# gt1/daccord

Measured on AMD Instinct MI355X. Metric: corrected Mbase/s (whole node), synthetic 20x PacBio piles, higher is better.
Workload: dtype u64+f64

## Files before the change

### daccord_amd/csrc/capi.hip

```cpp
#include <hip/hip_runtime.h>
#include <vector>
#include <string>
#include <cstring>
#include <cstdio>
#include <cstdlib>
#include <new>
#include "../../include/daccord_hip.h"
#include "batch_plan.hpp"
#include "host_tables.hpp"
#include "window_kernels.hpp"
#include "trace_kernel.hpp"
#include "vote_kernel.hpp"
#include "emit_record.hpp"

using namespace dacc;


struct PrepBatch
{
	DevOvl const * ovl; uint64_t novl; uint8_t const * trace; uint32_t trace_bytes;
	uint32_t * blk_ovl; uint32_t * blk_b0;
};

__global__ void k_prep(PrepBatch B)
// ... 528 lines not shown
		WB.pregen = 0;
		for ( uint32_t i = 0; i < TIER_NSTAGES; ++i ) c->st[i].ran = false;
		if ( TP.usefast && TP.anytier() )
		{
			HIPCHK(hipMemsetAsync(c->d_pregen.p,0,((BP.nwindows+31)/32+1)*sizeof(uint32_t),s));
			HIPCHK(hipMemsetAsync(c->d_pregen2.p,0,((BP.nwindows+31)/32+1)*sizeof(uint32_t),s));
			HIPCHK(hipMemsetAsync(c->d_pregenlist.p,0,sizeof(uint32_t),s));
			for ( int i = 0; i < TIER_NSLOTS; ++i ) HIPCHK(hipMemsetAsync(c->d_retry[i].p,0,sizeof(uint32_t),s));
			if ( BP.ovl.size() )
			{
				hipLaunchKernelGGL(k_prescan,dim3((BP.ovl.size()+3)/4),dim3(256),0,s,c->d_ovl.p,static_cast<uint64_t>(BP.ovl.size()),c->d_ovl_pile.p,c->d_piles.p,c->d_wt_b.p,c->d_wt_e.p,c->d_pregen.p,c->d_pregen2.p,TP.widetier ? 128u : 64u);
				hipLaunchKernelGGL(k_prescan_lists,dim3(((BP.nwindows+31)/32+255)/256),dim3(256),0,s,c->d_pregen.p,c->d_pregen2.p,static_cast<uint64_t>(BP.nwindows),c->d_pregenlist.p,
					TP.slot1_long ? c->d_retry[0].p : static_cast<uint32_t *>(0),c->d_wout.p);
			}
			HIPCHK(hipEventRecord(c->evPrescan,s));
			FastBatch FL; FL.W = WB; FL.W.arena = c->d_arena2.p; FL.W.prof = 0; FL.W.pregen = 0; FL.F = BP.ftierL; FL.dpsq_vst = c->d_vst.p; FL.retry = 0; FL.gearly = 0; FL.gslab = 0; FL.gstride = 0; FL.tab32 = c->d_tab32.p; FL.hand = 0; FL.handctr = 0; FL.handcap = 0; FL.handwords = 0;
#if defined(DACC_LEDGER)
			FL.ledger = 0;
#endif
			if ( !TP.ok[ID_LONG] ) FL.F.ldsbytes = 0;
			auto const launchLong = [&](uint32_t const * const lst, uint32_t & nlist, hipEvent_t const filled) -> int
			{
				nlist = 0;
				HIPCHK(hipStreamWaitEvent(c->stream2,filled,0));
				HIPCHK(hipMemcpyAsync(&nlist,lst,sizeof(uint32_t),hipMemcpyDeviceToHost,c->stream2));
				HIPCHK(hipStreamSynchronize(c->stream2));
				if ( !nlist ) return DACC_OK;
				uint32_t const grid = nlist < c->early_grid ? nlist : c->early_grid;
				(void)hipGetLastError();
				hipLaunchKernelGGL(k_window_long,dim3(grid),dim3(64),FL.F.ldsbytes,c->stream2,FL,c->d_err.p,lst);
				if ( FL.F.ldsbytes && hipGetLastError() != hipSuccess )
// ... 8 lines not shown
			HIPCHK(hipMemsetAsync(c->d_gearly.p,0,sizeof(uint32_t),s));
			HIPCHK(hipMemsetAsync(c->d_handctr.p,0,sizeof(uint32_t),s));
			bool early = false;
			HIPCHK(hipMemsetAsync(c->d_work.p,0,WORK_WORDS*sizeof(uint32_t),s));
			auto const work = [&](uint32_t const off) { return (c->sched&1) ? c->d_work.p+off : static_cast<uint32_t *>(0); };
			uint32_t const * list = 0; int lastslot = -1;
			FastBatch FZ;
			for ( uint32_t slot = 0; slot < TIER_NSLOTS; ++slot )
			{
				if ( TP.slotok(slot) )
				{
					int const m = TIER_MAIN[slot];
					FastBatch FB; FB.W = WB; FB.F = BP.stageCaps(m); FB.dpsq_vst = c->d_vst.p; FB.retry = c->d_retry[slot].p;
					if ( (slot > 0 && TP.late_long) || TP.widetier ) FB.W.pregen = c->d_pregen2.p;
					FB.gslab = c->d_gslab.p; FB.gstride = FB.F.gbytes; FB.tab32 = c->d_tab32.p;
					FB.hand = c->handcap ? c->d_hand.p : static_cast<uint64_t *>(0); FB.handctr = c->d_handctr.p; FB.handcap = c->handcap; FB.handwords = TP.handwords;
#if defined(DACC_LEDGER)
					{ char const * lm = getenv("DACC_LEDGER_MASK"); FB.ledger = lm ? static_cast<uint32_t>(strtoul(lm,0,0)) : 0u; }
#endif
					FB.gearly = early ? static_cast<uint32_t *>(0) : c->d_gearly.p;
					int fr[TIER_NSTAGES]; uint32_t nfr = 0;
					for ( int i = 0; i < m; ++i ) if ( TIER_CHAIN[i].slot == slot && TP.ok[i] && !((TIER_CHAIN[i].flags & STAGE_ADAPTIVE) && c->tier7_adapt_off) ) fr[nfr++] = i;
					bool const classed = nfr && (TIER_CHAIN[fr[0]].flags & STAGE_PREPASS);
					if ( classed ) HIPCHK(hipMemsetAsync(c->d_small.p,0,sizeof(uint32_t),s));
					for ( uint32_t k = 0; k < nfr; ++k ) HIPCHK(hipMemsetAsync(c->st[fr[k]].handon.p,0,sizeof(uint32_t),s));
					uint32_t const * in = list;
					if ( classed )
					{
						uint32_t * const mid = c->st[fr[0]].handon.p, * const big = c->st[fr[nfr-1]].handon.p;
						hipLaunchKernelGGL(k_classify,dim3((BP.nwindows+255)/256),dim3(256),0,s,WB,c->d_small.p,mid,big,c->sw.t0inst,nfr > 1 ? c->sw.t7inst : 0u);
						if ( nfr > 1 ) { HIPCHK(hipMemcpyAsync(c->d_work.p+WORK_PRE_MID,mid,sizeof(uint32_t),hipMemcpyDeviceToDevice,s)); HIPCHK(hipMemcpyAsync(c->d_work.p+WORK_PRE_BIG,big,sizeof(uint32_t),hipMemcpyDeviceToDevice,s)); }
// ... 509 lines not shown
```

### daccord_amd/csrc/fast_window.hpp

```cpp
#ifndef DACC_FAST_WINDOW_HPP
#define DACC_FAST_WINDOW_HPP
#include "wave.hpp"
#include "dev_types.hpp"
#include "arena.hpp"
#include "window_main.hpp"
#include "tier_pipeline.hpp"
#include "emit_record.hpp"

namespace dacc {

enum { WS_RETRY = 4 };
enum { FNOPAR = 0xFF };
enum { FSEQCAP = 48 };

struct FSI { uint64_t w; uint16_t left, right, current, path; };
struct FCC { uint64_t w; uint32_t o, l; };

template<int TIER> struct FastTier;
#if !defined(DACC_RCH01)
#define DACC_RCH01 2
#endif
template<> struct FastTier<1> { typedef uint8_t id_t; typedef uint8_t sid_t; enum : uint32_t { smax = 250, gw = 1, wcapg = 1024, rch = DACC_RCH01, fch = 4, fnw = 2, fnc = 40, idmax = 250, rpstcap = 256, lstr = 64, maxs = 32, precap = 1024, ncap = 776, scap = 112, lcap = 960, wcap = 1024, rccap = 144, fcap = 192, siqcap = 56, blcap = 96, seqcap = 32, psiq = 8, consrow = 64, lscrids = 2048, wide = 0, mins = 0, gmem = 0 }; };
template<> struct FastTier<0> { typedef uint8_t id_t; typedef uint8_t sid_t; enum : uint32_t { smax = 250, gw = 1, wcapg = 768, rch = DACC_RCH01, fch = 4, fnw = 2, fnc = 32, idmax = 250, rpstcap = 256, lstr = 64, maxs = 28, precap = 576, ncap = 524, scap = 88, lcap = 640, wcap = 768, rccap = 96, fcap = 128, siqcap = 56, blcap = 96, seqcap = 32, psiq = 8, consrow = 64, lscrids = 2048, wide = 0, mins = 0, gmem = 0 }; };
template<> struct FastTier<7> { typedef uint8_t id_t; typedef uint8_t sid_t; enum : uint32_t { smax = 250, gw = 1, wcapg = 896, rch = DACC_RCH01, fch = 4, fnw = 2, fnc = 32, idmax = 250, rpstcap = 256, lstr = 64, maxs = 28, precap = 704, ncap = 640, scap = 104, lcap = 800, wcap = 896, rccap = 112, fcap = 148, siqcap = 56, blcap = 96, seqcap = 32, psiq = 8, consrow = 64, lscrids = 2048, wide = 0, mins = 0, gmem = 0 }; };
// ... 383 lines not shown
	static_assert(CT::gmem == 0 || CT::gw != 0,"a layout in device memory is the gw layout");
	return C;
}

struct FastBatch
{
	WindowBatch W;
	FastCaps F;
	uint64_t const * dpsq_vst;
	uint32_t * retry;
	uint32_t * gearly;
	uint8_t * gslab;
	uint64_t gstride;
	uint32_t const * tab32;
	uint64_t * hand; uint32_t * handctr; uint32_t handcap, handwords;
#if defined(DACC_LEDGER)
	uint32_t ledger;
#endif
};

template<typename CT>
DEV void fast_load_tables(FastLds<CT> const & L, uint32_t const nrows, uint32_t const nsup, DevTables const & T, uint64_t const * vst)
{
	int const lane = wv_lane();
	for ( uint32_t i = lane; i < nsup; i += WSZ ) { L.suplo8()[i] = T.suplo[i]; L.suphi8()[i] = T.suphi[i]; }
	wv_sync();
}

#if defined(DACC_LEDGER)
#define LEDGER_REP(bit) for ( uint32_t lrep_ = 0, lrn_ = 1u + ((ledger >> (bit)) & 1u); lrep_ < lrn_; ++lrep_ )
#define LEDGER_REPX(E,bit) for ( uint32_t lrep_ = 0, lrn_ = 1u + (((E).ledger >> (bit)) & 1u); lrep_ < lrn_; ++lrep_ )
#else
#define LEDGER_REP(bit)
#define LEDGER_REPX(E,bit)
#endif
#define FW_THRES_FEAS 4294968ull
#define FW_THRES_01   429496730ull
#define FW_THRES_05   2147483648ull

#if defined(DACC_EMUL)
struct FastStats { uint32_t v[32]; void clear() { for ( int i = 0; i < 32; ++i ) v[i] = 0; } void mx(int i, uint32_t x) { if ( x > v[i] ) v[i] = x; } void add(int i, uint32_t x) { v[i] += x; } };
static FastStats g_fstats;
static inline void fstats_dump(int const tier)
{
	static FILE * sf = 0; static bool tried = false;
	if ( !tried ) { tried = true; char const * fn = getenv("DACC_EMUL_STATS"); if ( fn ) sf = fopen(fn,"w"); }
	if ( sf ) { fprintf(sf,"%d",tier); for ( int i = 0; i < 32; ++i ) fprintf(sf," %u",g_fstats.v[i]); fprintf(sf,"\n"); fflush(sf); }
}
static inline FILE * ftrav_file() { static FILE * f = 0; static bool tried = false; if ( !tried ) { tried = true; char const * fn = getenv("DACC_EMUL_TRAV"); if ( fn ) f = fopen(fn,"w"); } return f; }
#define FSTAT_MX(i,x) g_fstats.mx(i,x)
#define FSTAT_ADD(i,x) g_fstats.add(i,x)
#include <vector>
#include <algorithm>
struct FeasIters { std::vector<uint32_t> it, ln; void clear() { it.clear(); ln.clear(); } };
static FeasIters g_feasit;
static inline void feasit_dump()
{
	static FILE * f = 0; static bool tried = false;
	if ( !tried ) { tried = true; char const * fn = getenv("DACC_EMUL_FEAS"); if ( fn ) f = fopen(fn,"w"); }
	if ( !f ) { g_feasit.clear(); return; }
	std::vector<uint32_t> const & it = g_feasit.it; std::vector<uint32_t> const & ln = g_feasit.ln;
	uint64_t tot = 0, lock = 0, locksorted = 0;
// ... 33 lines not shown
	enum : bool { GW = (CT::gw != 0) };
	uint8_t * gslab;
	uint32_t const * gtab;
	struct G4 { uint32_t x, y, z, w; };
	int lane; uint32_t flags;
#if defined(DACC_LEDGER)
	uint32_t ledger;
#endif
	uint64_t * prof;
	uint32_t mao, k; uint64_t kmask;
	uint32_t npre, nlast, nn, nmfirst, nmlast;
	uint32_t n0, npool, nlinks, nwF, nwR;
	uint32_t nF, nL;

#if defined(DACC_EMUL)
	DEV void over_(uint32_t b, int line) { flags |= b; static char const * ov = getenv("DACC_EMUL_OVER"); if ( ov ) fprintf(stderr,"[over] tier maxs=%d line %d bits 0x%x nn=%u n0=%u npool=%u nF=%u nL=%u nwF=%u nwR=%u rstop=%u\n",int(CT::maxs)*10000+int(CT::ncap),line,b,nn,n0,npool,nF,nL,nwF,nwR,rstop); }
	#define over(b) over_(b,__LINE__)
#else
	DEV void over(uint32_t b) { flags |= b; }
#endif
#if defined(DACC_PROFILE) && !defined(DACC_EMUL)
	DEV void pcount(int id, uint64_t v) { if ( prof ) atomicAdd(reinterpret_cast<unsigned long long *>(prof+id),static_cast<unsigned long long>(v)); }
	DEV uint64_t pclock() { return clock64(); }
#else
	DEV void pcount(int, uint64_t) {}
	DEV uint64_t pclock() { return 0; }
#endif

#if defined(DACC_PROFILE) && !defined(DACC_EMUL)
	#define SITE_T0 uint64_t _ps = clock64();
	#define SITE_RESET { _ps = clock64(); }
// ... 32 lines not shown
		for ( uint32_t q = L.succ0()[z]; q < nn; ++q )
		{
			uint32_t const x = L.nv()[q];
			if ( x == target ) return q;
			if ( x > target ) break;
		}
		return -1;
	}
	DEV uint32_t nsucc(uint32_t z) const { return (L.sinfo()[z]>>8)&7; }
	DEV uint32_t nsuccact(uint32_t z) const { return (L.sinfo()[z]>>11)&7; }

	DEV void buildInstances()
	{
		PROFX_T0
		enum { NCH = (CT::maxs+WSZ-1)/WSZ };
#if defined(DACC_GEN_MARKS_NONE)
		enum : bool { GENMARKS = false };
#else
		enum : bool { GENMARKS = true };
#endif
		enum : bool { WIDES = FastLds<CT>::wides };
		enum : uint32_t { CLB = WIDES ? 10u : 8u, CLMASK = (1u << CLB) - 1u };
		static_assert(4u*CT::maxs <= FastLds<CT>::icap && CT::maxs <= (1u << CLB) && FastLds<CT>::icap <= (1u << (WIDES ? 16 : 24)),"compact string list: string | first slot << CLB, in the bytes of irpos");
		static_assert(!WIDES || GENMARKS,"the two-pass generation of more than 256 strings needs the marks");
		LDSQ uint8_t * const marks = L.ipos();
		LDSQ uint32_t * const clist = reinterpret_cast<LDSQ uint32_t *>(L.irpos());
		enum { NCHR = WIDES ? 1 : NCH };
		uint32_t nkc[NCHR], offc[NCHR], rkc[NCHR]; uint32_t base = 0, nl = 0;
		if constexpr ( WIDES )
		{
// ... 138 lines not shown
				p0 += dacc_popc64(m0); p1 += dacc_popc64(m1); p2 += dacc_popc64(m2); p3 += dacc_popc64(m3);
			}
			wv_sync();
			wv_sort_keys<CT::precap>(L.pre(),cnt0);
			wv_sort_keys<CT::precap>(L.pre()+o1,cnt1);
			wv_sort_keys<CT::precap>(L.pre()+o2,cnt2);
			wv_sort_keys<CT::precap>(L.pre()+o3,cnt3);
		}
		else
		wv_sort_keys<CT::precap,(CT::precap == 2048 && CT::ncap == 256)>(L.pre(),npre);
		SITE(33)
	}

	DEV void buildNodes(uint32_t const f)
	{
		uint32_t base = 0;
		for ( uint32_t c = 0; c < npre; c += WSZ )
		{
			uint32_t const i = c + lane;
			uint32_t keep = 0, e = i;
			if ( i < npre && (i == 0 || (L.pre()[i]>>32) != (L.pre()[i-1]>>32)) )
			{
				uint64_t const km = L.pre()[i]>>32;
				e = i+1;
				while ( e < npre && (L.pre()[e]>>32) == km ) ++e;
				keep = (e-i) >= f;
			}
			uint32_t tot; uint32_t const pre = wv_scan_excl(keep,tot);
			if ( keep )
			{
				uint32_t const z = base+pre;
				if ( z < CT::ncap ) { L.nv()[z] = static_cast<uint32_t>(L.pre()[i]>>32); L.nps()[z] = i; L.nfreq()[z] = (e-i) > FastLds<CT>::fqmax ? FastLds<CT>::fqmax : (e-i); if ( (e-i) > FastLds<CT>::fqmax ) over(2); }
			}
			base += tot;
		}
		nn = base;
		if ( nn > CT::ncap ) { over(2); nn = 0; }
		for ( uint32_t i = lane; i < npre; i += WSZ )
		{
			uint32_t const pos = (L.pre()[i]>>16)&0xFFFF, seq = L.pre()[i]&0xFFFF;
			uint32_t const rpos = L.slen()[seq]-pos-k;
			L.ipos()[i] = pos < nsup ? pos : nsup; L.irpos()[i] = rpos < nsup ? rpos : nsup;
		}
		wv_sync();
		if ( lane == 0 ) L.nps()[nn] = npre;
		for ( uint32_t z = lane; z < nn; z += WSZ )
		{
			uint32_t const s0 = L.nps()[z], f2 = L.nfreq()[z];
			uint32_t const lo = L.ipos()[s0], hi = L.ipos()[s0+f2-1];
			uint32_t rlo = 255, rhi = 0;
			for ( uint32_t q = 0; q < f2; ++q ) { uint32_t const r = L.irpos()[s0+q]; rlo = r < rlo ? r : rlo; rhi = r > rhi ? r : rhi; }
			uint32_t const pf = lo < nsup ? L.suplo8()[lo] : nrows, pt = hi < nsup ? L.suphi8()[hi] : nrows;
// ... 3 lines not shown
		uint32_t const kp2 = next_pow2(CT::maxs < 2 ? 2 : CT::maxs);
		base = 0;
		for ( uint32_t c = 0; c < nn; c += WSZ )
		{
			uint32_t const z = c + lane;
			uint32_t c0 = 0;
			if ( z < nn ) { uint32_t const s = L.nps()[z]; for ( uint32_t q = 0; q < L.nfreq()[z] && L.ipos()[s+q] == 0; ++q ) ++c0; }
			uint32_t tot; uint32_t const pre = wv_scan_excl(c0 ? 1 : 0,tot);
			if ( c0 && base+pre < kp2 ) L.mfirst()[base+pre] = ~((static_cast<uint64_t>(c0)<<32) | L.nv()[z]);
			base += tot;
		}
		nmfirst = base;
		if ( nmfirst > kp2 ) { over(8); nmfirst = 0; }
		uint32_t const p2 = next_pow2(nmfirst < 2 ? 2 : nmfirst);
		for ( uint32_t i = nmfirst + lane; i < p2; i += WSZ ) L.mfirst()[i] = ~0ull;
		base = 0;
		for ( uint32_t c = 0; c < nlast; c += WSZ )
		{
			uint32_t const i = c + lane;
			uint32_t const head = (i < nlast) && (i == 0 || (L.lastk()[i]>>32) != (L.lastk()[i-1]>>32));
			uint32_t tot; uint32_t const pre = wv_scan_excl(head,tot);
			if ( head )
			{
				uint32_t e = i+1;
				while ( e < nlast && (L.lastk()[e]>>32) == (L.lastk()[i]>>32) ) ++e;
				L.mlast()[base+pre] = ~((static_cast<uint64_t>(e-i)<<32) | (L.lastk()[i]>>32));
			}
			base += tot;
		}
		nmlast = base;
		uint32_t const q2 = next_pow2(nmlast < 2 ? 2 : nmlast);
		for ( uint32_t i = nmlast + lane; i < q2; i += WSZ ) L.mlast()[i] = ~0ull;
		wv_sync();
		wv_sort_keys<FastLds<CT>::keycap>(L.mfirst(),nmfirst);
		wv_sort_keys<FastLds<CT>::keycap>(L.mlast(),nmlast);
	}

	DEV void buildSuccessors(uint32_t const no)
	{
		uint32_t const lim = T.klim[(k-P.klow)*T.kln + (no < static_cast<uint32_t>(T.kln) ? no : T.kln-1)];
		for ( uint32_t z = lane; z < nn; z += WSZ )
		{
			uint32_t const masked = static_cast<uint32_t>((static_cast<uint64_t>(L.nv()[z])<<2) & kmask);
			uint32_t const s0 = lowerNode(masked);
			uint32_t k0 = 0, k1 = 0, k2 = 0, k3 = 0, n = 0;
			for ( uint32_t q = s0; q < nn && L.nv()[q] <= (masked|3); ++q )
			{
				uint32_t const kv = (static_cast<uint32_t>(L.nfreq()[q])<<8) | (L.nv()[q]&3);
				if ( n == 0 ) k0 = kv; else if ( n == 1 ) k1 = kv; else if ( n == 2 ) k2 = kv; else k3 = kv;
				++n;
// ... 15 lines not shown
			L.sinfo()[z] = order | (n<<8) | (act<<11);
		}
		wv_sync();
		sfresh = true;
	}
	DEV bool passIsDead() const
	{
		if ( nmfirst == 0 || nmlast == 0 ) return true;
		uint32_t const lastthres = ((static_cast<uint32_t>((~L.mlast()[0])>>32))*3)/4;
		uint32_t any = 0;
		for ( uint32_t i = lane; i < nmlast; i += WSZ )
		{
			uint64_t const e = ~L.mlast()[i];
			if ( static_cast<uint32_t>(e>>32) >= lastthres && findNode(static_cast<uint32_t>(e)) >= 0 ) any = 1;
		}
		return !wv_any(any);
	}
	DEV bool addNextFromHeap()
	{
		uint32_t best = 0;
		for ( uint32_t z = lane; z < nn; z += WSZ )
			if ( nsuccact(z) < nsucc(z) )
			{
				uint32_t const fq = L.nfreq()[succNode(z,nsuccact(z))];
				best = fq > best ? fq : best;
			}
		best = wv_max(best);
		if ( ! best ) return false;
		for ( uint32_t z = lane; z < nn; z += WSZ )
		{
// ... 76 lines not shown
		base = 0;
		for ( uint32_t c = 0; c < nane; c += WSZ )
		{
			uint32_t const i = c + lane;
			uint32_t ok = 0; uint32_t seqid = 0, pos = 0; uint64_t cv = 0;
			if ( i < nane )
			{
				pos = ANE[i]&0xFF; cv = ANE[i]>>8;
				for ( uint32_t j = 0; j < mao; ++j ) if ( pos + k <= L.slen()[j] ) { seqid = j; ok = 1; break; }
			}
			uint32_t tot; uint32_t const pre = wv_scan_excl(ok,tot);
			if ( ok && npre+base+pre < CT::precap ) L.pre()[npre+base+pre] = (cv<<32) | (static_cast<uint64_t>(pos)<<16) | seqid;
			base += tot;
		}
		if ( npre + base > CT::precap ) { over(1); return; }
		npre += base;
		wv_sync();
		wv_sort_keys<CT::precap>(L.pre(),npre);
	}

	DEV LDSQ uint16_t * stepTable() const { return L.xstep(); }
	DEV void computePredCounts()
	{
		LDSQ uint32_t * const cnt32 = L.xcnt32();
		LDSQ uint16_t * const stepT = stepTable();
		for ( uint32_t z = lane; 4u*z < nn; z += WSZ ) cnt32[z] = 0;
		wv_sync();
		for ( uint32_t u = lane; u < nn; u += WSZ )
		{
			uint32_t const na = nsuccact(u);
			uint32_t first = 0xFFFF;
// ... 87 lines not shown
		if ( nlinks > CT::lcap ) { over(64); n0 = 0; return; }
		wv_sync();
		for ( uint32_t q = lane; q < ns; q += WSZ )
		{
			uint32_t const len = L.tslen()[q]; uint64_t const sk = L.skey()[q];
			LDSQ uint16_t * const dst = L.links() + L.tlink()[q];
			if ( q < nslot && len <= WSLOT )
			{
				if constexpr ( GW ) { uint16_t const * src = reinterpret_cast<uint16_t const *>(gslab) + q*WSLOT; for ( uint32_t t = 0; t < len; ++t ) dst[t] = src[t]; }
				else { LDSQ uint16_t const * src = L.xwtmp() + q*WSLOT; for ( uint32_t t = 0; t < len; ++t ) dst[t] = src[t]; }
			}
			else { uint32_t ln; walkStretch(L.tfirst()[q],static_cast<uint32_t>(sk>>32),dst,ln); }
			L.tlast()[q] = static_cast<uint32_t>(sk);
		}
		wv_sync();
		uint32_t const p2 = next_pow2(ns < 2 ? 2 : ns);
		for ( uint32_t q = lane; q < p2; q += WSZ )
			L.skey()[q] = q < ns ? ((sortKey(L.tfirst()[q],L.links()[L.tlink()[q]+1],L.tslen()[q] < KFMAX ? L.tslen()[q] : KFMAX,L.tlast()[q])<<QB) | q) : ~0ull;
		wv_sync();
		wv_sort_keys<fcpow2(CT::scap)>(L.skey(),ns);
		uint32_t dup = 0;
		for ( uint32_t q = lane; q < ns; q += WSZ )
		{
			if ( q && (L.skey()[q]>>(QB+2*KF)) == (L.skey()[q-1]>>(QB+2*KF)) ) dup = 1;
			uint32_t const raw = L.skey()[q]&QMASK;
			L.sfirst()[q] = L.tfirst()[raw]; L.slast()[q] = L.tlast()[raw]; L.sslen()[q] = L.tslen()[raw]; L.slink()[q] = L.tlink()[raw];
		}
		if ( wv_any(dup) ) { over(32); n0 = 0; return; }
		n0 = ns;
		wv_sync();
		for ( uint32_t z = lane; z < nn; z += WSZ ) { L.npred()[z] = SNONE; L.lhead()[z] = SNONE; }
		for ( uint32_t q = lane; q < p2; q += WSZ ) L.skey()[q] = q < ns ? ((static_cast<uint64_t>(L.slast()[q])<<SB) | q) : ~0ull;
		wv_sync();
		for ( uint32_t q = lane; q < ns; q += WSZ ) if ( q == 0 || L.sfirst()[q-1] != L.sfirst()[q] ) L.npred()[L.sfirst()[q]] = q;
		wv_sort_keys<fcpow2(CT::scap)>(L.skey(),ns);
		for ( uint32_t q = lane; q < ns; q += WSZ )
		{
			uint64_t const e = L.skey()[q];
			L.lord()[q] = static_cast<uint32_t>(e);
			if ( q == 0 || (L.skey()[q-1]>>SB) != (e>>SB) ) L.lhead()[e>>SB] = q;
		}
		wv_sync();
	}

	DEV void makePiece(uint32_t const id, uint32_t const par, uint32_t const a, uint32_t const b)
	{
		LDSQ uint16_t const * Lk = L.links() + L.slink()[par];
		L.sfirst()[id] = Lk[a]; L.slast()[id] = Lk[b]; L.sslen()[id] = b-a+1; L.slink()[id] = L.slink()[par]+a;
	}
	DEV void findCandidatesAndPieces()
	{
		uint32_t const firstthres = nmfirst ? ((static_cast<uint32_t>((~L.mfirst()[0])>>32))*3)/4 : 0;
		uint32_t const lastthres = nmlast ? ((static_cast<uint32_t>((~L.mlast()[0])>>32))*3)/4 : 0;
		uint32_t cf = 0, cl = 0;
		while ( cf < nmfirst && static_cast<uint32_t>((~L.mfirst()[cf])>>32) >= firstthres ) ++cf;
		while ( cl < nmlast && static_cast<uint32_t>((~L.mlast()[cl])>>32) >= lastthres ) ++cl;
		nF = cf; npool = n0;
// ... 31 lines not shown
			{
				uint32_t const len = L.sslen()[s]; LDSQ uint16_t const * Lk = L.links() + L.slink()[s];
				for ( uint32_t i = 1; i+1 < len; ++i ) if ( sid[Lk[i]] != s ) multi = 1;
			}
			for ( uint32_t c = lane; c < nF; c += WSZ ) { uint32_t const z = L.fnode()[c]; if ( z != 0xFFFF && sid[z] != 0xFFFF ) { L.parF()[c] = sid[z]; L.posF()[c] = spos[z]; } }
			for ( uint32_t c = lane; c < nL; c += WSZ ) { uint32_t const z = L.lnode()[c]; if ( z != 0xFFFF && sid[z] != 0xFFFF ) { L.parL()[c] = sid[z]; L.posL()[c] = spos[z]; } }
		}
		if ( wv_any(multi) ) { over(32); return; }
		wv_sync();
		{
			uint32_t cnt = 0;
			for ( uint32_t c = 0; c < nF; ++c ) cnt += (L.parF()[c] != SNONE);
			for ( uint32_t c = 0; c < nL; ++c ) cnt += (L.parL()[c] != SNONE);
			if ( n0 + 2*cnt + 1 > CT::scap || n0 + 2*cnt + 1 > SMAX ) { over(32); return; }
		}
		{
			uint32_t id = n0;
			for ( uint32_t c0 = 0; c0 < nF + nL; c0 += WSZ )
			{
				uint32_t const c = c0 + lane;
				bool const isF = c < nF, act = c < nF + nL;
				uint32_t const ci = isF ? c : c - nF;
				uint32_t const par = act ? (isF ? L.parF()[ci] : L.parL()[ci]) : static_cast<uint32_t>(SNONE);
				bool const has = act && par != SNONE;
				uint32_t tot; uint32_t const pre = wv_scan_flag(has,tot);
				if ( has )
				{
					uint32_t const pid = id + 2*pre, pos = isF ? L.posF()[ci] : L.posL()[ci];
					if ( isF ) L.pieF()[ci] = pid; else L.pieL()[ci] = pid;
					makePiece(pid,par,0,pos); makePiece(pid+1,par,pos,L.sslen()[par]-1);
// ... 29 lines not shown
							while ( m < nm && !(L.midpar()[m] == pf && L.midA()[m] == lo && L.midB()[m] == hi) ) ++m;
							if ( m < nm ) continue;
							if ( nm < MIDCAP ) { L.midpar()[nm] = pf; L.midA()[nm] = lo; L.midB()[nm] = hi; }
							++nm;
						}
					}
				}
				wv_sync();
				nm = wv_bcast(nm,0);
				if ( nm > MIDCAP || npool + nm > CT::scap || npool + nm > SMAX ) { over(32); return; }
				for ( uint32_t m = lane; m < nm; m += WSZ ) makePiece(npool+m,L.midpar()[m],L.midA()[m],L.midB()[m]);
				nmid = nm; npool += nm;
				wv_sync();
			}
		}
		for ( uint32_t id = n0 + lane; id < npool; id += WSZ ) L.ppos()[id] = basePos(id);
		wv_sync();

	}

	DEV bool pairReachable()
	{
		LDSQ uint8_t * const seedN = L.xreach();
		LDSQ uint8_t * const reachN = seedN + CT::ncap;
		LDSQ uint8_t * const vis = reachN + CT::ncap;
		if ( nF == 0 || nL == 0 ) return false;
		for ( uint32_t z = lane; z < nn; z += WSZ ) { seedN[z] = 0; reachN[z] = 0; }
		for ( uint32_t s = lane; s < n0; s += WSZ ) vis[s] = 0;
		wv_sync();
		for ( uint32_t c = lane; c < nF; c += WSZ )
		{
			uint32_t const z = L.fnode()[c], par = L.parF()[c];
// ... 1457 lines not shown
			{
				uint64_t e0 = 0, e1 = 0, e2 = 0, e3 = 0;
				uint32_t const lo = 64*wq, hi = m < lo+64 ? m : lo+64;
				for ( uint32_t i = lo; i < hi; ++i )
				{
					uint32_t const c = s[i]; uint64_t const b = 1ull<<(i-lo);
					e0 |= (c == 0) ? b : 0; e1 |= (c == 1) ? b : 0; e2 |= (c == 2) ? b : 0; e3 |= (c == 3) ? b : 0;
				}
				L.peq()[4*PW*j+0*PW+wq] = e0; L.peq()[4*PW*j+1*PW+wq] = e1; L.peq()[4*PW*j+2*PW+wq] = e2; L.peq()[4*PW*j+3*PW+wq] = e3;
			}
		}
		wv_sync();
	}

	bool sfresh, sdirty;
	DEV void spillS()
	{
		if constexpr ( GW )
		{
			typedef FastLds<CT> LL;
			constexpr uint32_t plen = ((LL::upool - LL::sbase + 15u) & ~15u) < LL::sbytes ? ((LL::upool - LL::sbase + 15u) & ~15u) : LL::sbytes;
			constexpr uint32_t si0 = (LL::o_sinfo - LL::sbase) & ~15u, si1 = ((LL::e_sinfo - LL::sbase + 15u) & ~15u) < plen ? ((LL::e_sinfo - LL::sbase + 15u) & ~15u) : plen;
			LDSQ G4 const * const src = reinterpret_cast<LDSQ G4 const *>(L.base + LL::sbase);
			G4 * const dst = reinterpret_cast<G4 *>(gslab + LL::g_spill);
			wv_sync();
			if ( sfresh ) { for ( uint32_t i = lane; i < plen/16u; i += WSZ ) dst[i] = src[i]; }
			else if ( sdirty && si0 < si1 ) { for ( uint32_t i = si0/16u + lane; i < si1/16u; i += WSZ ) dst[i] = src[i]; }
			sfresh = false; sdirty = false;
			wv_sync();
		}
// ... 19 lines not shown
		sl = wv_bcast(sl,0);
		if ( !sl ) return 0;
		uint64_t * const dst = FB.hand + static_cast<uint64_t>(sl-1)*FB.handwords;
		if ( lane == 0 ) { dst[0] = npre | (static_cast<uint64_t>(nlast)<<32); dst[1] = k; }
		uint32_t const po = 2, lo = 2 + ((npre+1)&~1u);
		for ( uint32_t i = lane; i < npre; i += WSZ ) dst[po+i] = L.pre()[i];
		for ( uint32_t i = lane; i < nlast; i += WSZ ) dst[lo+i] = L.lastk()[i];
		return sl;
	}
	DEV bool loadHand(FastBatch const & FB, uint32_t const hslot)
	{
		uint64_t const * const src = FB.hand + static_cast<uint64_t>(hslot-1)*FB.handwords;
		uint64_t const h0 = src[0];
		uint32_t const n = static_cast<uint32_t>(h0), nl = static_cast<uint32_t>(h0>>32);
		if ( n > FastLds<CT>::icap || nl > FastLds<CT>::keycap || src[1] != k ) return false;
		npre = n; nlast = nl;
		FSTAT_ADD(31,1);
		uint32_t const po = 2, lo = 2 + ((n+1)&~1u);
		wv_sync();
		for ( uint32_t i = lane; i < n; i += WSZ ) L.pre()[i] = src[po+i];
		for ( uint32_t i = lane; i < nl; i += WSZ ) L.lastk()[i] = src[lo+i];
		wv_sync();
		return true;
	}
	DEV void restoreInstances()
	{
		if constexpr ( GW )
		{
			typedef FastLds<CT> LL;
			G4 const * const src = reinterpret_cast<G4 const *>(gslab + LL::g_inst);
			LDSQ G4 * const dp = reinterpret_cast<LDSQ G4 *>(L.pre());
// ... 705 lines not shown
	return 1u;
}

template<typename CT>
DEV int processWindowFast(FastBatch const & FB, uint64_t const widx, LDSQ uint8_t * lds, bool const resume = false)
{
	WindowBatch const & B = FB.W;
	FastEngine<CT> E;
#if defined(DACC_EMUL)
	{ char const * pz = getenv("DACC_EMUL_POISON"); if ( pz ) __builtin_memset(static_cast<void *>(&E),atoi(pz),sizeof(E)); }
#endif
	if ( B.pregen && ((B.pregen[widx>>5] >> (widx&31)) & 1) ) return FW_DONE;
	E.mao = 0; E.k = 0; E.kmask = 0; E.npre = E.nlast = E.nn = E.nmfirst = E.nmlast = 0; E.n0 = E.npool = E.nlinks = E.nwF = E.nwR = 0; E.nF = E.nL = 0;
	E.nsiq = E.ncdh = E.nacc = 0; E.rstop = 0; E.roundT0 = 0; E.cfree = 0; E.pvpath = E.pvrp = E.pvnf = 0; E.pvcl = 0; E.nmid = 0; E.midbase = 0; E.nLmagic = 0;
	E.T = B.T; E.P = B.P; E.nrows = FB.F.nrows; E.nsup = FB.F.nsup; E.vst = FB.dpsq_vst;
	E.gslab = 0; E.gtab = FB.tab32; E.sfresh = true; E.sdirty = false;
	if ( CT::gw )
	{
#if defined(DACC_EMUL)
		E.gslab = FB.gslab;
#else
		E.gslab = FB.gslab + static_cast<uint64_t>(blockIdx.x)*FB.gstride;
#endif
	}
	E.lane = wv_lane(); E.flags = 0; E.prof = B.prof;
#if defined(DACC_LEDGER)
	E.ledger = FB.ledger;
#endif
#if defined(DACC_PROFILE) && !defined(DACC_EMUL)
	uint64_t * const prof = E.prof;
#endif
// ... 5 lines not shown
	int const lane = E.lane;
	PROF_T0
	int32_t curff = B.P.maxff;
	uint32_t hslot = 0;
	bool const handable = FB.hand != 0 && B.P.klow == B.P.khigh && CT::gw != 0;
	if ( resume && B.P.klow == B.P.khigh )
	{
		WindowOut const prev = B.wout[widx];
		if ( prev.status == WS_RETRY && prev.filterfreq <= B.P.maxff && prev.filterfreq >= B.P.minff )
		{
			curff = prev.filterfreq;
			if ( handable && prev.minrate <= FB.handcap ) hslot = static_cast<uint32_t>(prev.minrate);
		}
	}
	int32_t const startff = curff;
	#define FFAIL(code) { if ( lane == 0 ) { B.wout[widx].status = WS_RETRY; B.wout[widx].flags = ((code)<<24) | (E.flags & 0xFFFFFF); B.wout[widx].filterfreq = curff; B.wout[widx].minrate = hslot; } return ((code) == 1 || (code) == 4) ? FW_GENERIC : FW_NEXT; }

	uint32_t lo = 0, hi = B.npiles;
	while ( hi-lo > 1 ) { uint32_t const mid = (lo+hi)>>1; if ( B.piles[mid].winbase <= widx ) lo = mid; else hi = mid; }
	DevPile const pile = B.piles[lo];
	uint32_t const y = static_cast<uint32_t>(widx - pile.winbase);
	uint32_t astart, aend;
	windowInterval(pile.l,B.P.a,B.P.w,y,astart,aend);

	WindowOut out; out.status = WS_INSUFFICIENT; out.mao = 0; out.elength = 0; out.k = 0; out.filterfreq = -1; out.conslen = 0; out.minrate = 0; out.flags = 0;
	uint8_t * rec = B.wrec + widx*(CT::wide ? DACC_WREC_OF(B.P.w) : static_cast<uint32_t>(WREC));
	if ( lane == 0 ) rec[0] = 0;
	if ( B.P.w > (CT::wide ? 127u : 63u) ) { FFAIL(1) }

	DevOvl const * ov = B.ovl + pile.first_ovl;
// ... 105 lines not shown
			bool instvalid = false, instsaved = false, handloaded = false;
			for ( int32_t ff = startff; ff >= B.P.minff; --ff )
			{
				curff = ff;
				PROF_T0
				if ( !instvalid )
				{
					SITE_T0
					if ( instsaved ) { E.restoreInstances(); SITE(27) }
					else if ( !(hslot && !handloaded && E.loadHand(FB,hslot)) ) { LEDGER_REPX(E,2) E.buildInstances(); SITE(28) }
					else { SITE(30) }
					handloaded = true;
				}
				if ( E.flags ) { FFAIL(7) }
				PROF(E,2)
				LEDGER_REPX(E,3) E.buildNodes(ff > 1 ? ff : 1);
				E.flags = wv_or(E.flags);
				if ( E.flags ) { if ( handable ) hslot = E.saveHand(FB,hslot); FFAIL(7) }
				PROF(E,3)
				instvalid = false;
				{ bool dead_ = false; LEDGER_REPX(E,16) dead_ = (ff != 0 && E.passIsDead()); if ( dead_ ) { instvalid = true; continue; } }
				if ( CT::gw != 0 && ff > B.P.minff && !instsaved ) { SITE_T0 LEDGER_REPX(E,17) E.saveInstances(); instsaved = true; SITE(29) }
				LEDGER_REPX(E,4) E.buildSuccessors(mao);
				PROF(E,4)
				if ( ff == 0 )
				{
					E.loadTab();
					E.levelSuccessors2();
					E.flags = wv_or(E.flags);
					if ( E.flags ) { FFAIL(6) }
// ... 84 lines not shown
```

### daccord_amd/csrc/tier_pipeline.hpp

```cpp
#ifndef DACC_TIER_PIPELINE_HPP
#define DACC_TIER_PIPELINE_HPP
#include <cstdint>
#include <cstdlib>
#include <algorithm>

namespace dacc {

struct FastCaps
{
	uint32_t maxs, precap, ncap, scap, lcap, wcap, rccap, fcap, siqcap, blcap;
	uint32_t tabcap;
	uint32_t nrows, nsup;
	uint32_t ldsbytes;
	uint32_t gbytes;
	uint32_t gmem;
};
enum { FSUPCAP = 128, FSUPCAPW = 192 };
enum : uint32_t { T0INST_DEFAULT = 576, T7INST_DEFAULT = 704 };

#define DACC_KERNEL_TIERS(X) X(0) X(1) X(2) X(3) X(4) X(6) X(7) X(8) X(9) X(10) X(11) X(12) X(13) X(14) X(15)
#define DACC_ALL_TIERS(X) DACC_KERNEL_TIERS(X) X(5)

template<int TIER> struct FastTier;
template<int TIER> struct TierTag { typedef FastTier<TIER> type; };
// ... 41 lines not shown
	{ { 3, 3, 9 }, 2, ROLE_MAIN, 2, GATE_TABFIT, WORK_SLOT2 },
	{ { 13, 13, 14 }, 2, ROLE_LAST, -1, GATE_TABFIT|GATE_LAST, WORK_LAST },
	{ { 15, 15, TIER_NONE }, 2, ROLE_LAST, -1, GATE_TABFIT|GATE_VDEEP, WORK_VDEEP },
	{ { 5, 5, TIER_NONE }, 0, ROLE_LONG, 2, GATE_TABFIT, 0 } };
static TierId const TIER_MAIN[TIER_NSLOTS] = { ID_SLOT0, ID_SLOT1, ID_SLOT2 };
static inline bool stageRuns(TierStage const & st, bool const deep, bool const wide) { return st.tier[wide ? 2 : deep] != TIER_NONE; }
static inline bool lastAsSlot2() { char const * const e = getenv("DACC_LAST_AS_SLOT2"); return e && e[0] == '1'; }
static inline bool vdeepAsSlot2() { char const * const e = getenv("DACC_VDEEP_AS_SLOT2"); return e && e[0] == '1'; }
static inline uint32_t stageTier(TierStage const & st, bool const deep, bool const wide)
{
	bool const slot2 = &st == &TIER_CHAIN[ID_SLOT2];
	TierStage const & t = (slot2 && lastAsSlot2()) ? TIER_CHAIN[ID_LAST] : ((slot2 && !wide && vdeepAsSlot2()) ? TIER_CHAIN[ID_VDEEP] : st);
	return (wide && t.tier[2] != TIER_NONE) ? t.tier[2] : (t.tier[deep] != TIER_NONE ? t.tier[deep] : t.tier[0]);
}

struct TierSwitches
{
	bool nofast;
	uint32_t tiers;
	bool widetier;
	bool dense;
	bool deepwin;
	bool lasttier;
	bool last_as_slot2;
	bool vdeeptier;
	bool vdeep_as_slot2;
	bool conflict() const { return last_as_slot2 && vdeep_as_slot2; }
	bool long128;
	bool hand;
	uint32_t t0inst, t7inst;
	uint32_t lds_t1, lds_t0;
};
static inline TierSwitches readTierSwitches()
{
	auto const off = [](char const * const name) { char const * const e = getenv(name); return e && e[0] == '0'; };
	auto const num = [](char const * const name, uint32_t const dflt) { char const * const e = getenv(name); return e ? static_cast<uint32_t>(atoi(e)) : dflt; };
	TierSwitches S;
	{ char const * const e = getenv("DACC_NOFAST"); S.nofast = e && e[0] == '1'; }
	S.tiers = num("DACC_TIERS",31);
	S.widetier = !off("DACC_WIDE_TIER"); S.dense = !off("DACC_DENSE_TIER"); S.deepwin = !off("DACC_DEEP_TIER"); S.lasttier = !off("DACC_LAST_TIER"); S.last_as_slot2 = lastAsSlot2(); S.vdeeptier = !off("DACC_VDEEP_TIER"); S.vdeep_as_slot2 = vdeepAsSlot2(); S.long128 = !off("DACC_LONG128"); S.hand = !off("DACC_HAND");
	S.t0inst = num("DACC_T0INST",T0INST_DEFAULT); S.t7inst = num("DACC_T7INST",T7INST_DEFAULT);
	S.lds_t1 = num("DACC_LDS_T1",0); S.lds_t0 = num("DACC_LDS_T0",0);
	return S;
}

enum : uint32_t { TIER_LDS_CU = 160*1024 };
static inline uint32_t tierGrid(uint32_t const ldsbytes, uint64_t const nwindows)
{
	uint64_t const percu = std::min<uint64_t>(8,std::max<uint64_t>(1,TIER_LDS_CU / (ldsbytes ? ldsbytes : 1)));
	return static_cast<uint32_t>(std::min<uint64_t>(256*percu,std::max<uint64_t>(8,((nwindows+7)/8)*8)));
}

enum : uint64_t { TIER_GMEM_SLAB = 256ull << 20 };
static inline uint32_t tierGridGmem(uint32_t const gbytes, uint64_t const nwindows)
{
// ... 56 lines not shown
```

Before: 39.48.

## Skip dead filter-frequency passes early and reuse last-key sort across passes

```diff
diff --git a/daccord_amd/csrc/capi.hip b/daccord_amd/csrc/capi.hip
--- a/daccord_amd/csrc/capi.hip
+++ b/daccord_amd/csrc/capi.hip
@@ -566,7 +566,7 @@
 					TP.slot1_long ? c->d_retry[0].p : static_cast<uint32_t *>(0),c->d_wout.p);
 			}
 			HIPCHK(hipEventRecord(c->evPrescan,s));
-			FastBatch FL; FL.W = WB; FL.W.arena = c->d_arena2.p; FL.W.prof = 0; FL.W.pregen = 0; FL.F = BP.ftierL; FL.dpsq_vst = c->d_vst.p; FL.retry = 0; FL.gearly = 0; FL.gslab = 0; FL.gstride = 0; FL.tab32 = c->d_tab32.p; FL.hand = 0; FL.handctr = 0; FL.handcap = 0; FL.handwords = 0;
+			FastBatch FL; FL.W = WB; FL.W.arena = c->d_arena2.p; FL.W.prof = 0; FL.W.pregen = 0; FL.F = BP.ftierL; FL.dpsq_vst = c->d_vst.p; FL.retry = 0; FL.gearly = 0; FL.gslab = 0; FL.gstride = 0; FL.tab32 = c->d_tab32.p; FL.hand = 0; FL.handctr = 0; FL.handcap = 0; FL.handwords = 0; FL.early = c->sw.early ? 1u : 0u;
 #if defined(DACC_LEDGER)
 			FL.ledger = 0;
 #endif
@@ -605,7 +605,7 @@
 					FastBatch FB; FB.W = WB; FB.F = BP.stageCaps(m); FB.dpsq_vst = c->d_vst.p; FB.retry = c->d_retry[slot].p;
 					if ( (slot > 0 && TP.late_long) || TP.widetier ) FB.W.pregen = c->d_pregen2.p;
 					FB.gslab = c->d_gslab.p; FB.gstride = FB.F.gbytes; FB.tab32 = c->d_tab32.p;
-					FB.hand = c->handcap ? c->d_hand.p : static_cast<uint64_t *>(0); FB.handctr = c->d_handctr.p; FB.handcap = c->handcap; FB.handwords = TP.handwords;
+					FB.hand = c->handcap ? c->d_hand.p : static_cast<uint64_t *>(0); FB.handctr = c->d_handctr.p; FB.handcap = c->handcap; FB.handwords = TP.handwords; FB.early = c->sw.early ? 1u : 0u;
 #if defined(DACC_LEDGER)
 					{ char const * lm = getenv("DACC_LEDGER_MASK"); FB.ledger = lm ? static_cast<uint32_t>(strtoul(lm,0,0)) : 0u; }
 #endif
diff --git a/daccord_amd/csrc/fast_window.hpp b/daccord_amd/csrc/fast_window.hpp
--- a/daccord_amd/csrc/fast_window.hpp
+++ b/daccord_amd/csrc/fast_window.hpp
@@ -421,6 +421,7 @@
 	uint64_t gstride;
 	uint32_t const * tab32;
 	uint64_t * hand; uint32_t * handctr; uint32_t handcap, handwords;
+	uint32_t early = 1;
 #if defined(DACC_LEDGER)
 	uint32_t ledger;
 #endif
@@ -446,13 +447,15 @@
 #define FW_THRES_05   2147483648ull
 
 #if defined(DACC_EMUL)
-struct FastStats { uint32_t v[32]; void clear() { for ( int i = 0; i < 32; ++i ) v[i] = 0; } void mx(int i, uint32_t x) { if ( x > v[i] ) v[i] = x; } void add(int i, uint32_t x) { v[i] += x; } };
+static uint64_t g_fstats_total[72];
+struct FastStats { uint32_t v[40]; void clear() { for ( int i = 0; i < 40; ++i ) v[i] = 0; } void mx(int i, uint32_t x) { if ( x > v[i] ) v[i] = x; } void add(int i, uint32_t x) { v[i] += x; g_fstats_total[i] += x; } };
 static FastStats g_fstats;
+extern "C" inline __attribute__((used,visibility("default"))) void dacc_emul_fstats_total(uint64_t * const out) { for ( int i = 0; i < 72; ++i ) out[i] = g_fstats_total[i]; }
 static inline void fstats_dump(int const tier)
 {
 	static FILE * sf = 0; static bool tried = false;
 	if ( !tried ) { tried = true; char const * fn = getenv("DACC_EMUL_STATS"); if ( fn ) sf = fopen(fn,"w"); }
-	if ( sf ) { fprintf(sf,"%d",tier); for ( int i = 0; i < 32; ++i ) fprintf(sf," %u",g_fstats.v[i]); fprintf(sf,"\n"); fflush(sf); }
+	if ( sf ) { fprintf(sf,"%d",tier); for ( int i = 0; i < 40; ++i ) fprintf(sf," %u",g_fstats.v[i]); fprintf(sf,"\n"); fflush(sf); }
 }
 static inline FILE * ftrav_file() { static FILE * f = 0; static bool tried = false; if ( !tried ) { tried = true; char const * fn = getenv("DACC_EMUL_TRAV"); if ( fn ) f = fopen(fn,"w"); } return f; }
 #define FSTAT_MX(i,x) g_fstats.mx(i,x)
@@ -516,7 +519,7 @@
 	uint32_t nF, nL;
 
 #if defined(DACC_EMUL)
-	DEV void over_(uint32_t b, int line) { flags |= b; static char const * ov = getenv("DACC_EMUL_OVER"); if ( ov ) fprintf(stderr,"[over] tier maxs=%d line %d bits 0x%x nn=%u n0=%u npool=%u nF=%u nL=%u nwF=%u nwR=%u rstop=%u\n",int(CT::maxs)*10000+int(CT::ncap),line,b,nn,n0,npool,nF,nL,nwF,nwR,rstop); }
+	DEV void over_(uint32_t b, int line) { flags |= b; for ( int i = 0; i < 32; ++i ) if ( (b >> i) & 1u ) ++g_fstats_total[40+i]; static char const * ov = getenv("DACC_EMUL_OVER"); if ( ov ) fprintf(stderr,"[over] tier maxs=%d line %d bits 0x%x nn=%u n0=%u npool=%u nF=%u nL=%u nwF=%u nwR=%u rstop=%u\n",int(CT::maxs)*10000+int(CT::ncap),line,b,nn,n0,npool,nF,nL,nwF,nwR,rstop); }
 	#define over(b) over_(b,__LINE__)
 #else
 	DEV void over(uint32_t b) { flags |= b; }
@@ -579,6 +582,7 @@
 	{
 		PROFX_T0
 		enum { NCH = (CT::maxs+WSZ-1)/WSZ };
+		posvalid = false;
 #if defined(DACC_GEN_MARKS_NONE)
 		enum : bool { GENMARKS = false };
 #else
@@ -747,6 +751,7 @@
 
 	DEV void buildNodes(uint32_t const f)
 	{
+		FSTAT_ADD(32,1);
 		uint32_t base = 0;
 		for ( uint32_t c = 0; c < npre; c += WSZ )
 		{
@@ -769,6 +774,7 @@
 		}
 		nn = base;
 		if ( nn > CT::ncap ) { over(2); nn = 0; }
+		if ( !posvalid )
 		for ( uint32_t i = lane; i < npre; i += WSZ )
 		{
 			uint32_t const pos = (L.pre()[i]>>16)&0xFFFF, seq = L.pre()[i]&0xFFFF;
@@ -802,6 +808,8 @@
 		if ( nmfirst > kp2 ) { over(8); nmfirst = 0; }
 		uint32_t const p2 = next_pow2(nmfirst < 2 ? 2 : nmfirst);
 		for ( uint32_t i = nmfirst + lane; i < p2; i += WSZ ) L.mfirst()[i] = ~0ull;
+		if ( !posvalid )
+		{
 		base = 0;
 		for ( uint32_t c = 0; c < nlast; c += WSZ )
 		{
@@ -819,9 +827,11 @@
 		nmlast = base;
 		uint32_t const q2 = next_pow2(nmlast < 2 ? 2 : nmlast);
 		for ( uint32_t i = nmlast + lane; i < q2; i += WSZ ) L.mlast()[i] = ~0ull;
+		}
 		wv_sync();
 		wv_sort_keys<FastLds<CT>::keycap>(L.mfirst(),nmfirst);
-		wv_sort_keys<FastLds<CT>::keycap>(L.mlast(),nmlast);
+		if ( !posvalid ) { FSTAT_ADD(34,1); wv_sort_keys<FastLds<CT>::keycap>(L.mlast(),nmlast); }
+		posvalid = poskeep;
 	}
 
 	DEV void buildSuccessors(uint32_t const no)
@@ -867,6 +877,52 @@
 			uint64_t const e = ~L.mlast()[i];
 			if ( static_cast<uint32_t>(e>>32) >= lastthres && findNode(static_cast<uint32_t>(e)) >= 0 ) any = 1;
 		}
+		return !wv_any(any);
+	}
+	DEV bool passDeadOnInstances(uint32_t const f) const
+	{
+		if ( nsup == 0 || f == 0 ) return false;
+		if ( nlast == 0 ) return false;
+		uint32_t cnt = 0, first = 0, big = 0;
+		for ( uint32_t i = lane; i < npre; i += WSZ )
+		{
+			uint64_t const w = L.pre()[i];
+			uint32_t const km = static_cast<uint32_t>(w>>32);
+			bool const head = i == 0 || static_cast<uint32_t>(L.pre()[i-1]>>32) != km;
+			if ( head && i+f-1 < npre && static_cast<uint32_t>(L.pre()[i+f-1]>>32) == km )
+			{
+				++cnt;
+				first |= ((static_cast<uint32_t>(w)>>16) == 0) ? 1u : 0u;
+				big |= (i+FastLds<CT>::fqmax < npre && static_cast<uint32_t>(L.pre()[i+FastLds<CT>::fqmax]>>32) == km) ? 1u : 0u;
+			}
+		}
+		cnt = wv_sum(cnt);
+		if ( wv_any(big) || cnt > CT::ncap ) return false;
+		if ( !wv_any(first) ) return true;
+		uint32_t best = 0;
+		for ( uint32_t i = lane; i < nlast; i += WSZ )
+			if ( i == 0 || (L.lastk()[i]>>32) != (L.lastk()[i-1]>>32) )
+			{
+				uint32_t e = i+1;
+				while ( e < nlast && (L.lastk()[e]>>32) == (L.lastk()[i]>>32) ) ++e;
+				best = (e-i) > best ? (e-i) : best;
+			}
+		best = wv_max(best);
+		uint32_t const lastthres = (best*3)/4;
+		uint32_t any = 0;
+		for ( uint32_t i = lane; i < nlast; i += WSZ )
+			if ( i == 0 || (L.lastk()[i]>>32) != (L.lastk()[i-1]>>32) )
+			{
+				uint32_t const km = static_cast<uint32_t>(L.lastk()[i]>>32);
+				uint32_t e = i+1;
+				while ( e < nlast && static_cast<uint32_t>(L.lastk()[e]>>32) == km ) ++e;
+				if ( (e-i) >= lastthres )
+				{
+					uint32_t lo = 0, hi = npre;
+					while ( lo < hi ) { uint32_t const mid = (lo+hi)>>1; if ( static_cast<uint32_t>(L.pre()[mid]>>32) < km ) lo = mid+1; else hi = mid; }
+					if ( lo+f-1 < npre && static_cast<uint32_t>(L.pre()[lo]>>32) == km && static_cast<uint32_t>(L.pre()[lo+f-1]>>32) == km ) any = 1;
+				}
+			}
 		return !wv_any(any);
 	}
 	DEV bool addNextFromHeap()
@@ -973,7 +1029,7 @@
 			base += tot;
 		}
 		if ( npre + base > CT::precap ) { over(1); return; }
-		npre += base;
+		npre += base; posvalid = false;
 		wv_sync();
 		wv_sort_keys<CT::precap>(L.pre(),npre);
 	}
@@ -1091,6 +1147,8 @@
 			L.tlast()[q] = static_cast<uint32_t>(sk);
 		}
 		wv_sync();
+		LEDGER_REP(19)
+		{
 		uint32_t const p2 = next_pow2(ns < 2 ? 2 : ns);
 		for ( uint32_t q = lane; q < p2; q += WSZ )
 			L.skey()[q] = q < ns ? ((sortKey(L.tfirst()[q],L.links()[L.tlink()[q]+1],L.tslen()[q] < KFMAX ? L.tslen()[q] : KFMAX,L.tlast()[q])<<QB) | q) : ~0ull;
@@ -1118,6 +1176,7 @@
 			if ( q == 0 || (L.skey()[q-1]>>SB) != (e>>SB) ) L.lhead()[e>>SB] = q;
 		}
 		wv_sync();
+		}
 	}
 
 	DEV void makePiece(uint32_t const id, uint32_t const par, uint32_t const a, uint32_t const b)
@@ -1179,6 +1238,7 @@
 			for ( uint32_t c = 0; c < nL; ++c ) cnt += (L.parL()[c] != SNONE);
 			if ( n0 + 2*cnt + 1 > CT::scap || n0 + 2*cnt + 1 > SMAX ) { over(32); return; }
 		}
+		LEDGER_REP(20)
 		{
 			uint32_t id = n0;
 			for ( uint32_t c0 = 0; c0 < nF + nL; c0 += WSZ )
@@ -1238,8 +1298,8 @@
 				wv_sync();
 			}
 		}
-		for ( uint32_t id = n0 + lane; id < npool; id += WSZ ) L.ppos()[id] = basePos(id);
-		wv_sync();
+		LEDGER_REP(20) { for ( uint32_t id = n0 + lane; id < npool; id += WSZ ) L.ppos()[id] = basePos(id);
+		wv_sync(); }
 
 	}
 
@@ -2727,6 +2787,7 @@
 	}
 
 	bool sfresh, sdirty;
+	bool posvalid, poskeep;
 	DEV void spillS()
 	{
 		if constexpr ( GW )
@@ -2776,7 +2837,7 @@
 		uint64_t const h0 = src[0];
 		uint32_t const n = static_cast<uint32_t>(h0), nl = static_cast<uint32_t>(h0>>32);
 		if ( n > FastLds<CT>::icap || nl > FastLds<CT>::keycap || src[1] != k ) return false;
-		npre = n; nlast = nl;
+		npre = n; nlast = nl; posvalid = false;
 		FSTAT_ADD(31,1);
 		uint32_t const po = 2, lo = 2 + ((n+1)&~1u);
 		wv_sync();
@@ -3512,7 +3573,7 @@
 	E.mao = 0; E.k = 0; E.kmask = 0; E.npre = E.nlast = E.nn = E.nmfirst = E.nmlast = 0; E.n0 = E.npool = E.nlinks = E.nwF = E.nwR = 0; E.nF = E.nL = 0;
 	E.nsiq = E.ncdh = E.nacc = 0; E.rstop = 0; E.roundT0 = 0; E.cfree = 0; E.pvpath = E.pvrp = E.pvnf = 0; E.pvcl = 0; E.nmid = 0; E.midbase = 0; E.nLmagic = 0;
 	E.T = B.T; E.P = B.P; E.nrows = FB.F.nrows; E.nsup = FB.F.nsup; E.vst = FB.dpsq_vst;
-	E.gslab = 0; E.gtab = FB.tab32; E.sfresh = true; E.sdirty = false;
+	E.gslab = 0; E.gtab = FB.tab32; E.sfresh = true; E.sdirty = false; E.posvalid = false; E.poskeep = false;
 	if ( CT::gw )
 	{
 #if defined(DACC_EMUL)
@@ -3548,6 +3609,12 @@
 		}
 	}
 	int32_t const startff = curff;
+#if defined(DACC_EMUL)
+	bool const early = earlyPass();
+#else
+	bool const early = FB.early != 0;
+#endif
+	E.poskeep = early;
 	#define FFAIL(code) { if ( lane == 0 ) { B.wout[widx].status = WS_RETRY; B.wout[widx].flags = ((code)<<24) | (E.flags & 0xFFFFFF); B.wout[widx].filterfreq = curff; B.wout[widx].minrate = hslot; } return ((code) == 1 || (code) == 4) ? FW_GENERIC : FW_NEXT; }
 
 	uint32_t lo = 0, hi = B.npiles;
@@ -3683,6 +3750,7 @@
 				}
 				if ( E.flags ) { FFAIL(7) }
 				PROF(E,2)
+				if ( early && ff != 0 ) { bool dead_ = false; LEDGER_REPX(E,18) dead_ = E.passDeadOnInstances(static_cast<uint32_t>(ff)); if ( dead_ ) { FSTAT_ADD(33,1); instvalid = true; continue; } }
 				LEDGER_REPX(E,3) E.buildNodes(ff > 1 ? ff : 1);
 				E.flags = wv_or(E.flags);
 				if ( E.flags ) { if ( handable ) hslot = E.saveHand(FB,hslot); FFAIL(7) }
diff --git a/daccord_amd/csrc/tier_pipeline.hpp b/daccord_amd/csrc/tier_pipeline.hpp
--- a/daccord_amd/csrc/tier_pipeline.hpp
+++ b/daccord_amd/csrc/tier_pipeline.hpp
@@ -79,6 +79,7 @@
 	return (wide && t.tier[2] != TIER_NONE) ? t.tier[2] : (t.tier[deep] != TIER_NONE ? t.tier[deep] : t.tier[0]);
 }
 
+static inline bool earlyPass() { char const * const e = getenv("DACC_EARLY_PASS"); return !(e && e[0] == '0'); }
 struct TierSwitches
 {
 	bool nofast;
@@ -93,6 +94,7 @@
 	bool conflict() const { return last_as_slot2 && vdeep_as_slot2; }
 	bool long128;
 	bool hand;
+	bool early;
 	uint32_t t0inst, t7inst;
 	uint32_t lds_t1, lds_t0;
 };
@@ -103,7 +105,7 @@
 	TierSwitches S;
 	{ char const * const e = getenv("DACC_NOFAST"); S.nofast = e && e[0] == '1'; }
 	S.tiers = num("DACC_TIERS",31);
-	S.widetier = !off("DACC_WIDE_TIER"); S.dense = !off("DACC_DENSE_TIER"); S.deepwin = !off("DACC_DEEP_TIER"); S.lasttier = !off("DACC_LAST_TIER"); S.last_as_slot2 = lastAsSlot2(); S.vdeeptier = !off("DACC_VDEEP_TIER"); S.vdeep_as_slot2 = vdeepAsSlot2(); S.long128 = !off("DACC_LONG128"); S.hand = !off("DACC_HAND");
+	S.widetier = !off("DACC_WIDE_TIER"); S.dense = !off("DACC_DENSE_TIER"); S.deepwin = !off("DACC_DEEP_TIER"); S.lasttier = !off("DACC_LAST_TIER"); S.last_as_slot2 = lastAsSlot2(); S.vdeeptier = !off("DACC_VDEEP_TIER"); S.vdeep_as_slot2 = vdeepAsSlot2(); S.long128 = !off("DACC_LONG128"); S.hand = !off("DACC_HAND"); S.early = earlyPass();
 	S.t0inst = num("DACC_T0INST",T0INST_DEFAULT); S.t7inst = num("DACC_T7INST",T7INST_DEFAULT);
 	S.lds_t1 = num("DACC_LDS_T1",0); S.lds_t0 = num("DACC_LDS_T0",0);
 	return S;
```

Result: no change. 39.46 (-0.1%).
